# qazwsxal/diffusion-extensions

Measured on NVIDIA B200. Metric: igso3_score_evals_per_sec, higher is better.
Workload: dtype f32

## Files before the change

### diffusion_extensions_b200/csrc/so3d_kernels.cu

```cuda
#include <cuda_runtime.h>
#include <stdio.h>
#include <type_traits>
#include <stdlib.h>
#include <string.h>

#include "../../include/so3d.h"
#include "so3d_math.cuh"
#include "so3d_lanes.cuh"
#include "so3d_tma.cuh"
#include "so3d_cdf_smem.cuh"

using namespace so3d;

namespace {

constexpr int kTile = 256;

#ifndef SO3D_QS_OUTSTAGES
#define SO3D_QS_OUTSTAGES 1
#endif
#ifndef SO3D_QS_MINCTAS
#define SO3D_QS_MINCTAS 4
#endif
#ifndef SO3D_WROW_SHFL
// ... 1133 lines not shown
    float ga;
    aa_to_rmat_bwd(a3[0], angle[i], a9[0], &o3[0], &ga);
    g_angle[i] = ga;
  }
};
struct ExpVecBwdOp {
  SO3D_OP_ARRAYS(1, 1, 0, 1)
  SO3D_OP_NO_TAB
  __device__ void row(int64_t, const Mat3* a9, const Vec3* a3, Mat3*, Vec3* o3, const float*) const {
    o3[0] = exp_vec_bwd(a3[0], exp_vec(a3[0]), a9[0]);
  }
};
struct ScaleBwdOp {
  SO3D_OP_ARRAYS(2, 0, 1, 0)
  SO3D_OP_NO_TAB
  const float* s;
  int s_stride;
  float* g_s;
  __device__ void row(int64_t i, const Mat3* a9, const Vec3*, Mat3* o9, Vec3*, const float*) const {
    const float sc = s[i * s_stride];
    const Vec3 lv = log_vec(a9[0]);
    const Vec3 w{sc * lv.x, sc * lv.y, sc * lv.z};
    const Vec3 gw = exp_vec_bwd(w, exp_vec(w), a9[1]);
    if (g_s) g_s[i] = fmaf(lv.x, gw.x, fmaf(lv.y, gw.y, lv.z * gw.z));
    const Vec3 gl{0.5f * sc * gw.x, 0.5f * sc * gw.y, 0.5f * sc * gw.z};
    o9[0] = log_bwd(a9[0], hat(gl));
  }
};

#ifndef SO3D_LOGP_PREFETCH
#define SO3D_LOGP_PREFETCH 1
#endif
template <bool kOn>
struct LogpPre {};
template <>
struct LogpPre<true> {
  struct Pre1 {};
  struct Pre2 {
    float eps;
  };
};
template <int kMode>
struct LogpScoreOp : LogpPre<SO3D_LOGP_PREFETCH && (kMode == kClosed || kMode == kAuto)> {
  SO3D_OP_ARRAYS(1, 0, 0, 1)
  SO3D_OP_NO_TAB
  static constexpr int kMinCtas = (kMode == kClosed || kMode == kAuto) ? 5 : 1;
#ifndef SO3D_SERIES_WIDE_INDEX
#define SO3D_SERIES_WIDE_INDEX 0
#endif
  static constexpr bool kWideIndex = SO3D_SERIES_WIDE_INDEX && (kMode == kSeries || kMode == kSeriesAdaptive || kMode == kSeriesPure);
  const float* eps;
  int eps_stride;
  float* logp;
  float* dlogf;
  int L;
  __device__ void row(int64_t i, const Mat3* a9, const Vec3*, Mat3*, Vec3* o3, const float*) const { row_eps(i, eps[i * eps_stride], a9, o3); }
  __device__ void row_eps(int64_t i, float e, const Mat3* a9, Vec3* o3) const {
    const AxisAngleF a = axis_angle_fast(a9[0]);
    float lf, g;
    igso3_logf_g_t<kMode>(a.theta, e, L, &lf, &g);
    logp[i] = lf;
    if (dlogf) dlogf[i] = g;
    o3[0] = Vec3{g * a.axis.x, g * a.axis.y, g * a.axis.z};
  }
  template <class P1 = typename LogpPre<true>::Pre1>
  __device__ P1 prefetch1(int64_t) const { return P1{}; }
  template <class P1, class P2 = typename LogpPre<true>::Pre2>
  __device__ P2 prefetch2(int64_t i, const P1&) const { return P2{eps[i * eps_stride]}; }
  template <class P2>
  __device__ void row(int64_t i, const P2& p, const Mat3* a9, const Vec3*, Mat3*, Vec3* o3, const float*) const { row_eps(i, p.eps, a9, o3); }
};
#ifndef SO3D_LOGP2_MINCTAS
#define SO3D_LOGP2_MINCTAS 8
#endif
#ifndef SO3D_LOGP2_AUTO_VOTE
#define SO3D_LOGP2_AUTO_VOTE 1
#endif
#ifndef SO3D_LOGP2_OUTSTAGES
#define SO3D_LOGP2_OUTSTAGES 1
#endif
#ifndef SO3D_SERIES2_MINCTAS
#define SO3D_SERIES2_MINCTAS 4
#endif
template <int kMode>
struct LogpScore2Op : LogpScoreOp<kMode> {
  static constexpr bool kSeriesMode = kMode == kSeries || kMode == kSeriesAdaptive || kMode == kSeriesPure;
  using Pre1 = typename LogpPre<true>::Pre1;
  using Pre2 = typename LogpPre<true>::Pre2;
  static constexpr int kOutStages = SO3D_LOGP2_OUTSTAGES;
  static constexpr int kInStages = 1;
  static constexpr int kMinCtas = kSeriesMode ? SO3D_SERIES2_MINCTAS : SO3D_LOGP2_MINCTAS;
  int64_t n;
  __device__ void row2(int64_t i0, const Pre2 (&p)[2], const Mat3 (*a9)[2], const Vec3 (*)[2], Mat3 (*)[2], Vec3 (*o3)[2], const float*) const {
    const AxisAngleL<L2> a = axis_angle_fast_l(lanes_of(a9[0][0], a9[0][1]));
    float lf2[2], g2[2];
    if constexpr (kSeriesMode) {
      igso3_series_branch_l2<kMode>(a.theta, L2{p[0].eps, p[1].eps}, this->L, lf2, g2);
    } else if (kMode == kAuto && SO3D_LOGP2_AUTO_VOTE) {
      igso3_closed_f32(a.theta.x, p[0].eps, &lf2[0], &g2[0]);
      igso3_closed_f32(a.theta.y, p[1].eps, &lf2[1], &g2[1]);
      const bool s0 = !(p[0].eps <= kAutoSeriesEps), s1 = !(p[1].eps <= kAutoSeriesEps);
      if (__any_sync(__activemask(), s0 || s1)) {
        if (s0) igso3_series_branch<kAuto>(a.theta.x, p[0].eps, this->L, &lf2[0], &g2[0]);
        if (s1) igso3_series_branch<kAuto>(a.theta.y, p[1].eps, this->L, &lf2[1], &g2[1]);
      }
    } else {
      igso3_logf_g_t<kMode>(a.theta.x, p[0].eps, this->L, &lf2[0], &g2[0]);
      igso3_logf_g_t<kMode>(a.theta.y, p[1].eps, this->L, &lf2[1], &g2[1]);
    }
#pragma unroll
    for (int j = 0; j < 2; ++j) {
      const int64_t i = i0 + 32 * j;
      const float lf = lf2[j], g = g2[j];
      if (i < n) {
        this->logp[i] = lf;
        if (this->dlogf) this->dlogf[i] = g;
      }
      o3[0][j] = j ? Vec3{g * a.axis.x.y, g * a.axis.y.y, g * a.axis.z.y} : Vec3{g * a.axis.x.x, g * a.axis.y.x, g * a.axis.z.x};
    }
  }
};
struct LogpBwdOp {
  SO3D_OP_ARRAYS(1, 0, 1, 0)
  SO3D_OP_NO_TAB
  const float* dlogf;
  const float* gout;
  __device__ void row(int64_t i, const Mat3* a9, const Vec3*, Mat3* o9, Vec3*, const float*) const {
    const Mat3& r = a9[0];
    const float vx = r.m[7] - r.m[5], vy = r.m[2] - r.m[6], vz = r.m[3] - r.m[1];
    const float s = 0.5f * sqrtf(fmaf(vx, vx, fmaf(vy, vy, vz * vz)));
    const float c = 0.5f * (r.m[0] + r.m[4] + r.m[8] - 1.0f);
    const float gg = gout[i] * dlogf[i] / fmaf(s, s, c * c);
    const float ka = s > 0.f ? gg * c / (4.0f * s) : 0.f;
    const float kd = -0.5f * gg * s;
#pragma unroll
    for (int p = 0; p < 3; ++p)
#pragma unroll
      for (int q = 0; q < 3; ++q) o9[0].m[3 * p + q] = ka * (r.m[3 * p + q] - r.m[3 * q + p]) + (p == q ? kd : 0.f);
  }
};

__global__ void __launch_bounds__(256) density_kernel(const float* __restrict__ omega, const float* __restrict__ eps, int eps_stride,
                                                      float* __restrict__ f, int64_t n, int mode, int L) {
  for (int64_t i = (int64_t)blockIdx.x * blockDim.x + threadIdx.x; i < n; i += (int64_t)gridDim.x * blockDim.x) {
    float lf, g;
    igso3_logf_g(omega[i], eps[i * eps_stride], mode, L, &lf, &g);
    f[i] = expf(lf);
  }
}

template <int kMode>
__global__ void __launch_bounds__(256) series_warp_kernel(const float* __restrict__ R, const float* __restrict__ eps, int eps_stride,
                                                          float* __restrict__ logp, float* __restrict__ score3, float* __restrict__ dlogf,
                                                          int64_t n, int L) {
  const int lane = threadIdx.x & 31;
  const int64_t warps = ((int64_t)gridDim.x * blockDim.x) >> 5;
  for (int64_t row = ((int64_t)blockIdx.x * blockDim.x + threadIdx.x) >> 5; row < n; row += warps) {
    Mat3 m;
#pragma unroll
    for (int k = 0; k < 9; ++k) m.m[k] = __ldg(R + row * 9 + k);
    const AxisAngleF a = axis_angle_fast(m);
    const float e = __ldg(eps + row * eps_stride);
    float kap, kapp, cexp;
    igso3_series_lane_setup(a.theta, e, &kap, &kapp, &cexp);
    const int Lw = igso3_series_warp_terms(e, L);
    SeriesLaneState st = igso3_series_lane(kap, kapp, cexp, lane, igso3_series_lane_terms(Lw), Lw);
#pragma unroll
    for (int off = 16; off > 0; off >>= 1) {
      st.b += __shfl_xor_sync(0xffffffffu, st.b, off);
      st.d += __shfl_xor_sync(0xffffffffu, st.d, off);
      st.bp += __shfl_xor_sync(0xffffffffu, st.bp, off);
      st.dp += __shfl_xor_sync(0xffffffffu, st.dp, off);
    }
    if (lane == 0) {
      const float F = 2.0f * st.b - st.d, dF = 2.0f * st.bp - st.dp;
      float lf = logf(2.0f * F), g = dF / F;
      if ((kMode == kSeries || kMode == kSeriesAdaptive) && e <= kAutoSeriesEps && a.theta > kSeriesGuard * e) igso3_closed_f32(a.theta, e, &lf, &g);
      logp[row] = lf;
      if (dlogf) dlogf[row] = g;
      if (score3) {
// ... 1078 lines not shown
  op.in9[0] = R; op.q = q4;
  return launch_rowwise_pick(op, n, stream, "so3d_rmat_to_quat_f32");
}

}

template <bool TA, bool TB>
static int compose_dispatch(const float* A, int a_stride, const float* B, int b_stride, float* C, int64_t n, void* stream) {
  if (a_stride && b_stride) {
    ComposeOp<TA, TB> op;
    op.in9[0] = A; op.in9[1] = B; op.out9[0] = C;
    return launch_rowwise_pick(op, n, stream, "so3d_compose_f32");
  } else if (!a_stride && b_stride) {
    ComposeSharedOp<TA, TB, true> op;
    op.in9[0] = B; op.shared = A; op.out9[0] = C;
    return launch_rowwise_pick(op, n, stream, "so3d_compose_f32");
  } else if (a_stride && !b_stride) {
    ComposeSharedOp<TA, TB, false> op;
    op.in9[0] = A; op.shared = B; op.out9[0] = C;
    return launch_rowwise_pick(op, n, stream, "so3d_compose_f32");
  }
  return fail(SO3D_EINVAL, "so3d_compose_f32: at most one operand may be shared");
}

extern "C" {

int so3d_compose_f32(const float* A, int a_stride, int trans_a, const float* B, int b_stride, int trans_b, float* C,
                     int64_t n, void* stream) {
  SO3D_REQUIRE(n == 0 || (A && B && C), "so3d_compose_f32: null pointer");
  if (trans_a && trans_b) return compose_dispatch<true, true>(A, a_stride, B, b_stride, C, n, stream);
  if (trans_a) return compose_dispatch<true, false>(A, a_stride, B, b_stride, C, n, stream);
  if (trans_b) return compose_dispatch<false, true>(A, a_stride, B, b_stride, C, n, stream);
  return compose_dispatch<false, false>(A, a_stride, B, b_stride, C, n, stream);
}

int so3d_rmat_dist_f32(const float* A, const float* B, float* out, int64_t n, void* stream) {
  SO3D_REQUIRE(n == 0 || (A && B && out), "so3d_rmat_dist_f32: null pointer");
  RmatDistOp op;
  op.in9[0] = A; op.in9[1] = B; op.out = out;
  return launch_rowwise_pick(op, n, stream, "so3d_rmat_dist_f32", true);
}

int so3d_lerp_f32(const float* A, const float* B, const float* w, int w_stride, float* out, int64_t n, void* stream) {
  SO3D_REQUIRE(n == 0 || (A && B && w && out), "so3d_lerp_f32: null pointer");
  SO3D_REQUIRE(w_stride == 0 || w_stride == 1, "so3d_lerp_f32: w_stride must be 0 or 1");
  LerpOp op;
  op.in9[0] = A; op.in9[1] = B; op.w = w; op.w_stride = w_stride; op.out9[0] = out;
  return launch_rowwise_pick(op, n, stream, "so3d_lerp_f32");
}

int so3d_log_bwd_f32(const float* R, const float* G9, float* gR, int64_t n, void* stream) {
  SO3D_REQUIRE(n == 0 || (R && G9 && gR), "so3d_log_bwd_f32: null pointer");
  LogBwdOp op;
  op.in9[0] = R; op.in9[1] = G9; op.out9[0] = gR;
  return launch_rowwise_pick(op, n, stream, "so3d_log_bwd_f32");
}

int so3d_aa_to_rmat_bwd_f32(const float* axis3, const float* angle, const float* G9, float* g_axis3, float* g_angle,
                            int64_t n, void* stream) {
  SO3D_REQUIRE(n == 0 || (axis3 && angle && G9 && g_axis3 && g_angle), "so3d_aa_to_rmat_bwd_f32: null pointer");
  AaToRmatBwdOp op;
  op.in9[0] = G9; op.in3[0] = axis3; op.angle = angle; op.out3[0] = g_axis3; op.g_angle = g_angle;
  return launch_rowwise_pick(op, n, stream, "so3d_aa_to_rmat_bwd_f32");
}

int so3d_expvec_bwd_f32(const float* v3, const float* G9, float* g_v3, int64_t n, void* stream) {
  SO3D_REQUIRE(n == 0 || (v3 && G9 && g_v3), "so3d_expvec_bwd_f32: null pointer");
  ExpVecBwdOp op;
  op.in9[0] = G9; op.in3[0] = v3; op.out3[0] = g_v3;
  return launch_rowwise_pick(op, n, stream, "so3d_expvec_bwd_f32");
}

int so3d_scale_bwd_f32(const float* R, const float* s, int s_stride, const float* G9, float* gR, float* g_s, int64_t n,
                       void* stream) {
  SO3D_REQUIRE(n == 0 || (R && s && G9 && gR), "so3d_scale_bwd_f32: null pointer");
  SO3D_REQUIRE(s_stride == 0 || s_stride == 1, "so3d_scale_bwd_f32: s_stride must be 0 or 1");
  ScaleBwdOp op;
  op.in9[0] = R; op.in9[1] = G9; op.s = s; op.s_stride = s_stride; op.g_s = g_s; op.out9[0] = gR;
  return launch_rowwise_pick(op, n, stream, "so3d_scale_bwd_f32");
}

}

template <int kMode>
static int launch_logp_score(const float* R, const float* eps, int eps_stride, float* logp, float* score3, float* dlogf, int64_t n, int L,
                             void* stream) {
  constexpr bool kSeriesMode = LogpScore2Op<kMode>::kSeriesMode;
  if constexpr (kSeriesMode || SO3D_LOGP_PREFETCH) {
    const char* lanes_env = getenv("SO3D_LOGP_LANES");
    if (!(lanes_env && atoi(lanes_env) == 1)) {
      LogpScore2Op<kMode> op2;
      op2.in9[0] = R; op2.eps = eps; op2.eps_stride = eps_stride; op2.logp = logp; op2.dlogf = dlogf; op2.out3[0] = score3;
      op2.L = L; op2.n = n;
      return launch_rowwise_w2(op2, n, stream, "so3d_igso3_logp_score_f32", kMode == kSeriesAdaptive ? 3 : 0);
    }
  }
  LogpScoreOp<kMode> op;
  op.in9[0] = R; op.eps = eps; op.eps_stride = eps_stride; op.logp = logp; op.dlogf = dlogf; op.out3[0] = score3;
  op.L = L;
  const int ctas = (kMode == kSeries || kMode == kSeriesAdaptive || kMode == kSeriesPure) ? 3 : 0;
  return launch_rowwise(op, n, stream, "so3d_igso3_logp_score_f32", ctas);
}

extern "C" {

static int check_mode(int mode, int L) {
  if (mode < 0 || mode > 4) return fail(SO3D_EINVAL, "mode must be SO3D_MODE_{SERIES,CLOSED,AUTO,SERIES_ADAPTIVE,SERIES_PURE}");
  if (mode != SO3D_MODE_CLOSED && (L < 1 || L > 2896)) return fail(SO3D_EINVAL, "series truncation L must be in [1, 2896]");
  return 0;
}

int so3d_igso3_density_f32(const float* omega, const float* eps, int eps_stride, float* f, int64_t n, int mode, int L,
                           void* stream) {
  SO3D_REQUIRE(n >= 0, "negative n");
  if (n == 0) return 0;
  SO3D_REQUIRE(omega && eps && f, "so3d_igso3_density_f32: null pointer");
  SO3D_REQUIRE(eps_stride == 0 || eps_stride == 1, "eps_stride must be 0 or 1");
  if (int rc = check_mode(mode, L)) return rc;
  const int64_t blocks = (n + 255) / 256;
  const int64_t cap = (int64_t)sm_count() * 8;
  density_kernel<<<(int)(blocks < cap ? blocks : cap), 256, 0, (cudaStream_t)stream>>>(omega, eps, eps_stride, f, n, mode, L);
  return check_launch("so3d_igso3_density_f32");
}

int so3d_igso3_logp_score_f32(const float* R, const float* eps, int eps_stride, float* logp, float* score3, float* dlogf,
                              int64_t n, int mode, int L, void* stream) {
  SO3D_REQUIRE(n == 0 || (R && eps && logp), "so3d_igso3_logp_score_f32: null pointer");
  SO3D_REQUIRE(eps_stride == 0 || eps_stride == 1, "eps_stride must be 0 or 1");
  if (int rc = check_mode(mode, L)) return rc;
  if (n > 0 && (mode == SO3D_MODE_SERIES || mode == SO3D_MODE_SERIES_ADAPTIVE || mode == SO3D_MODE_SERIES_PURE)) {
    static const int64_t rows_per_sm = [] { const char* e = getenv("SO3D_SERIES_WARP_ROWS"); return e ? (int64_t)atoll(e) : (int64_t)64; }();
    if (n <= rows_per_sm * sm_count()) {
      const int64_t blocks = (n * 32 + 255) / 256;
      const int64_t cap = (int64_t)sm_count() * 8;
      const int grid = (int)(blocks < cap ? blocks : cap);
      if (mode == SO3D_MODE_SERIES_PURE)
        series_warp_kernel<kSeriesPure><<<grid, 256, 0, (cudaStream_t)stream>>>(R, eps, eps_stride, logp, score3, dlogf, n, L);
      else
        series_warp_kernel<kSeries><<<grid, 256, 0, (cudaStream_t)stream>>>(R, eps, eps_stride, logp, score3, dlogf, n, L);
      return check_launch("so3d_igso3_logp_score_f32");
    }
  }
  switch (mode) {
    case SO3D_MODE_SERIES: return launch_logp_score<kSeries>(R, eps, eps_stride, logp, score3, dlogf, n, L, stream);
    case SO3D_MODE_CLOSED: return launch_logp_score<kClosed>(R, eps, eps_stride, logp, score3, dlogf, n, L, stream);
    case SO3D_MODE_AUTO: return launch_logp_score<kAuto>(R, eps, eps_stride, logp, score3, dlogf, n, L, stream);
    case SO3D_MODE_SERIES_PURE: return launch_logp_score<kSeriesPure>(R, eps, eps_stride, logp, score3, dlogf, n, L, stream);
    default: return launch_logp_score<kSeriesAdaptive>(R, eps, eps_stride, logp, score3, dlogf, n, L, stream);
  }
}

int so3d_igso3_logp_bwd_f32(const float* R, const float* dlogf, const float* gout, float* gR, int64_t n, void* stream) {
  SO3D_REQUIRE(n == 0 || (R && dlogf && gout && gR), "so3d_igso3_logp_bwd_f32: null pointer");
  LogpBwdOp op;
  op.in9[0] = R; op.dlogf = dlogf; op.gout = gout; op.out9[0] = gR;
  return launch_rowwise_pick(op, n, stream, "so3d_igso3_logp_bwd_f32");
}

int so3d_igso3_cdf_table_f32(const float* eps, int64_t rows, const float* grid_loc, const float* haar_w, float* trap_out,
                             int quirks, void* stream) {
  SO3D_REQUIRE(rows >= 0, "negative rows");
  if (rows == 0) return 0;
  SO3D_REQUIRE(eps && grid_loc && haar_w && trap_out, "so3d_igso3_cdf_table_f32: null pointer");
  SO3D_REQUIRE(rows <= 0x7fffffff, "so3d_igso3_cdf_table_f32: too many rows");
  cdf_table_kernel<<<(int)rows, 256, 0, (cudaStream_t)stream>>>(eps, grid_loc, haar_w, trap_out, quirks);
  return check_launch("so3d_igso3_cdf_table_f32");
}

}

template <bool kShared>
static int launch_sample(const float* cdf, const uint32_t* guide, const float* loc, int64_t rows, const int64_t* row_idx, int64_t row,
                         const float* u, const float* axes3, uint64_t seed, uint64_t rng_offset, uint64_t row_offset, const float* mean,
                         int mean_stride, float* R, float* angle, float* axis3, int64_t n, void* stream) {
  SampleOp<kShared> op;
  op.out9[0] = R; op.out3[0] = axis3;
  op.cdf = cdf; op.guide = guide; op.loc = loc; op.row_idx = row_idx; op.shared_row = row; op.rows = rows; op.u_in = u; op.axes_in = axes3;
// ... 331 lines not shown
```

### diffusion_extensions_b200/csrc/so3d_lanes.cuh

```cuda
#pragma once

#include "so3d_math.cuh"

namespace so3d {

struct L1 {
  float x;
};
struct alignas(8) L2 {
  float x, y;
};
struct M1 {
  bool x;
};
struct M2 {
  bool x, y;
};
template <class L>
struct MaskOf;
template <>
struct MaskOf<L1> {
  using type = M1;
};
template <>
// ... 237 lines not shown
  const M pos = ge(n2, bc<L>(kFltMin));
  const L rs = sel(pos, vrsqrt(n2), zero);
  const L c = mulc(0.5f, add(add(add(r.m[0], r.m[4]), r.m[8]), bc<L>(-1.0f)));
  AxisAngleL<L> o;
  o.theta = atan2_pos_l(mul(mul(sel(tiny, bc<L>(0.5f * kTinyDown), bc<L>(0.5f)), n2), rs), c);
  const L d0 = sub(r.m[0], c), d1 = sub(r.m[4], c), d2 = sub(r.m[8], c);
  const L s01 = mulc(0.5f, add(r.m[1], r.m[3])), s02 = mulc(0.5f, add(r.m[2], r.m[6])), s12 = mulc(0.5f, add(r.m[5], r.m[7]));
  const M p0 = mand(ge(d0, d1), ge(d0, d2));
  const M p1 = ge(d1, d2);
  const L cx = sel(p0, d0, sel(p1, s01, s02));
  const L cy = sel(p0, s01, sel(p1, d1, s12));
  const L cz = sel(p0, s02, sel(p1, s12, d2));
  const L cn = vrsqrt(vmax(fma(cx, cx, fma(cy, cy, mul(cz, cz))), bc<L>(1e-30f)));
  const L sg = sel(lt(fma(cx, vx, fma(cy, vy, mul(cz, vz))), zero), neg(cn), cn);
  const M near_pi = lt(c, bc<L>(kNearPiCos));
  o.axis.x = sel(near_pi, mul(cx, sg), mul(vx, rs));
  o.axis.y = sel(near_pi, mul(cy, sg), mul(vy, rs));
  o.axis.z = sel(near_pi, mul(cz, sg), sel(mnot(pos), bc<L>(1.0f), mul(vz, rs)));
  return o;
}
template <class L>
SO3D_HD void quat_axis_halfangle_l(const QuatL<L>& q, Vec3L<L>* n, L* half) {
  using M = typename MaskOf<L>::type;
  const L zero = bc<L>(0.f);
  const M tiny = lt(fma(q.x, q.x, fma(q.y, q.y, mul(q.z, q.z))), bc<L>(kFltMin));
  const L sc = sel(tiny, bc<L>(kTinyUp), bc<L>(1.0f));
  const L x = mul(q.x, sc), y = mul(q.y, sc), z = mul(q.z, sc);
  const L v2 = fma(x, x, fma(y, y, mul(z, z)));
  const M pos = ge(v2, bc<L>(kFltMin));
  const L rs = sel(pos, vrsqrt(v2), zero);
  *half = atan2_pos_l(mul(mul(sel(tiny, bc<L>(kTinyDown), bc<L>(1.0f)), v2), rs), vabs(q.w));
  const L k = sel(lt(q.w, zero), neg(rs), rs);
  *n = Vec3L<L>{mul(x, k), mul(y, k), sel(pos, mul(z, k), bc<L>(1.0f))};
}

template <class L, bool kHasPred>
SO3D_HD QuatL<L> p_mean_quat_l(const Mat3L<L>& x_t, const Vec3L<L>& pred, float a, float b, float c1, float c2, QuatL<L>* x0h) {
  const AxisAngleL<L> ax = axis_angle_fast_l(x_t);
  QuatL<L> qh = quat_axis_angle_l(ax.axis, mulc(a, ax.theta));
  if (kHasPred) {
    const QuatL<L> q2 = quat_exp_vec_l(Vec3L<L>{mulc(-b, pred.x), mulc(-b, pred.y), mulc(-b, pred.z)});
    qh = qmul_l(qh, q2);
  }
  Vec3L<L> n0;
  L h0;
  quat_axis_halfangle_l(qh, &n0, &h0);
  const QuatL<L> q3 = quat_axis_angle_l(n0, mulc(2.0f * c1, h0));
  const QuatL<L> q4 = quat_axis_angle_l(ax.axis, mulc(c2, ax.theta));
  *x0h = qh;
  return qmul_l(q3, q4);
}

template <class L>
SO3D_HD QuatL<L> p_mean_quat_rows_l(const Mat3L<L>& x_t, const Vec3L<L>& pred, L a, L b, L c1, L c2, QuatL<L>* x0h) {
  const AxisAngleL<L> ax = axis_angle_fast_l(x_t);
  const L nb = neg(b);
  const QuatL<L> q1 = quat_axis_angle_l(ax.axis, mul(a, ax.theta));
  const QuatL<L> q2 = quat_exp_vec_l(Vec3L<L>{mul(nb, pred.x), mul(nb, pred.y), mul(nb, pred.z)});
  const QuatL<L> qh = qmul_l(q1, q2);
  Vec3L<L> n0;
  L h0;
  quat_axis_halfangle_l(qh, &n0, &h0);
  const QuatL<L> q3 = quat_axis_angle_l(n0, mul(mulc(2.0f, c1), h0));
  const QuatL<L> q4 = quat_axis_angle_l(ax.axis, mul(c2, ax.theta));
  *x0h = qh;
  return qmul_l(q3, q4);
}

SO3D_HD void sincos_draw_l(L1 x, L1* s, L1* c) { sincos_draw(x.x, &s->x, &c->x); }
SO3D_HD void sincos_draw_l(L2 x, L2* s, L2* c) {
  sincos_draw(x.x, &s->x, &c->x);
  sincos_draw(x.y, &s->y, &c->y);
}
template <class L>
SO3D_HD Vec3L<L> sphere_from_uniforms_l(L ua, L ub) {
  const L z = fma(bc<L>(-2.0f), ua, bc<L>(1.0f));
  const L t = mul(mulc(4.0f, ua), sub(bc<L>(1.0f), ua));
  const L r = mul(t, vrsqrt(vmax(t, bc<L>(1e-30f))));
  L sp, cp;
  sincos_draw_l(fma(bc<L>(kTwoPi), ub, bc<L>(-kPi)), &sp, &cp);
  return Vec3L<L>{mul(r, cp), mul(r, sp), z};
}

#ifndef SO3D_SERIES2_ORDER
#define SO3D_SERIES2_ORDER 0
#endif
#ifndef SO3D_SERIES2_BLOCK
#define SO3D_SERIES2_BLOCK 32
#endif
constexpr int kSeries2Block = SO3D_SERIES2_BLOCK;
struct SeriesStateL2 {
  L2 b, d, bp, dp, b2, bp2;
};
SO3D_HD L2 series_dsrc_l2(L2 kapp, L2 b, L2 dp) {
#if SO3D_SERIES_DERIV
  (void)kapp;
  return sub(dp, b);
#else
  return fnma(kapp, b, dp);
#endif
}
template <int kUnroll>
SO3D_HD void igso3_series_run_l2(SeriesStateL2& st, L2 kap, L2 kapp, L2 cexp, int hi, int count) {
#pragma unroll kUnroll
  for (int i = 0; i < count; ++i) {
    const int l = hi - i;
    const L2 e = vex2(mul(bc<L2>(series_mm(l)), cexp));
    const L2 mh = bc<L2>(series_mh(l));
    st.b2 = st.b;
    st.bp2 = st.bp;
#if SO3D_SERIES2_ORDER == 0
    const L2 dn = fnma(kap, st.b, fma(e, mh, st.d));
    const L2 dpn = fnma(kap, st.bp, series_dsrc_l2(kapp, st.b, st.dp));
    st.b = add(st.b, dn);
    st.bp = add(st.bp, dpn);
#elif SO3D_SERIES2_ORDER == 1
    const L2 t = fma(e, mh, st.d);
    const L2 u = series_dsrc_l2(kapp, st.b, st.dp);
    const L2 dn = fnma(kap, st.b, t);
    const L2 dpn = fnma(kap, st.bp, u);
    st.b = add(st.b, dn);
    st.bp = add(st.bp, dpn);
#elif SO3D_SERIES2_ORDER == 2
    const L2 dpn = fnma(kap, st.bp, series_dsrc_l2(kapp, st.b, st.dp));
    const L2 dn = fnma(kap, st.b, fma(e, mh, st.d));
    st.bp = add(st.bp, dpn);
    st.b = add(st.b, dn);
#else
    const L2 dn = fnma(kap, st.b, fma(e, mh, st.d));
    const L2 bn = add(st.b, dn);
    const L2 u = series_dsrc_l2(kapp, st.b, st.dp);
    const L2 dpn = fnma(kap, st.bp, u);
    st.b = bn;
    st.bp = add(st.bp, dpn);
#endif
    st.d = dn;
    st.dp = dpn;
  }
}

template <int kMode>
SO3D_HD void igso3_series_branch_l2(L2 w, L2 eps, int L, float* logf_out, float* g_out) {
  static_assert(kMode == kSeries || kMode == kSeriesAdaptive || kMode == kSeriesPure, "series modes only");
  int terms = L;
  if (kMode == kSeriesAdaptive) {
    const int t0 = igso3_series_live_terms(eps.x, L), t1 = igso3_series_live_terms(eps.y, L);
    terms = t0 > t1 ? t0 : t1;
#if defined(__CUDA_ARCH__)
    terms = __reduce_max_sync(__activemask(), terms);
#endif
#if SO3D_SERIES_ROUNDUP
    const int up = (terms + kSeries2Block - 1) / kSeries2Block * kSeries2Block;
    terms = up <= L ? up : L;
#endif
  }
  constexpr bool kGuarded = kMode != kSeriesPure;
  const bool guard0 = kGuarded && eps.x <= kAutoSeriesEps && w.x > kSeriesGuard * eps.x;
  const bool guard1 = kGuarded && eps.y <= kAutoSeriesEps && w.y > kSeriesGuard * eps.y;
  float lf_c[2] = {0.f, 0.f}, g_c[2] = {0.f, 0.f};
  if (guard0) igso3_closed_f32_outofline(w.x, eps.x, &lf_c[0], &g_c[0]);
  if (guard1) igso3_closed_f32_outofline(w.y, eps.y, &lf_c[1], &g_c[1]);
  L2 kap, kapp, cexp;
  igso3_series_lane_setup(w.x, eps.x, &kap.x, &kapp.x, &cexp.x);
  igso3_series_lane_setup(w.y, eps.y, &kap.y, &kapp.y, &cexp.y);
  const L2 zero = bc<L2>(0.f);
  SeriesStateL2 st{zero, zero, zero, zero, zero, zero};
  const int ragged = terms % kSeries2Block;
  if (ragged) igso3_series_run_l2<1>(st, kap, kapp, cexp, terms - 1, ragged);
  for (int blk = terms / kSeries2Block - 1; blk >= 0; --blk)
    igso3_series_run_l2<kSeries2Block>(st, kap, kapp, cexp, blk * kSeries2Block + (kSeries2Block - 1), kSeries2Block);
  const L2 F = add(st.b, st.b2);
#if SO3D_SERIES_DERIV
  const L2 dF = mul(kapp, add(st.bp, st.bp2));
#else
  const L2 dF = add(st.bp, st.bp2);
#endif
  logf_out[0] = guard0 ? lf_c[0] : logf(2.0f * F.x);
  g_out[0] = guard0 ? g_c[0] : dF.x / F.x;
  logf_out[1] = guard1 ? lf_c[1] : logf(2.0f * F.y);
  g_out[1] = guard1 ? g_c[1] : dF.y / F.y;
}

template <class L>
SO3D_HD QuatL<L> q_sample_quat_l(const Mat3L<L>& x0, L sc, const Vec3L<L>& axis, L ang, QuatL<L>* qn_out) {
  const QuatL<L> qn = quat_axis_angle_l(axis, ang);
  const AxisAngleL<L> ax = axis_angle_fast_l(x0);
  *qn_out = qn;
  return qmul_l(quat_axis_angle_l(ax.axis, mul(sc, ax.theta)), qn);
}

SO3D_HD Mat3L<L1> lanes_of(const Mat3& a) {
  Mat3L<L1> r;
  for (int k = 0; k < 9; ++k) r.m[k] = L1{a.m[k]};
  return r;
}
SO3D_HD Mat3L<L2> lanes_of(const Mat3& a, const Mat3& b) {
  Mat3L<L2> r;
  for (int k = 0; k < 9; ++k) r.m[k] = L2{a.m[k], b.m[k]};
  return r;
}

}
```

### profiles/sass_series_reads.py

```python
#!/usr/bin/env python
import argparse
import collections
import json
import os
import re
import subprocess
import sys

ROOT = os.path.dirname(os.path.dirname(os.path.abspath(__file__)))
sys.path.insert(0, ROOT)

WORDS_PER_CLK = 2.0
XU_CLK_PER_MUFU = 8.0
INS = re.compile(r"/\*([0-9a-f]{4,})\*/\s+(.*?)\s*;")
REG = re.compile(r"^-?\|?(R\d+)((?:\.\w+)*)\|?$")


def cuobjdump():
    from diffusion_extensions_b200 import build
    return os.path.join(os.path.dirname(build.find_nvcc()), "cuobjdump")


def functions(sass):
    out, cur = {}, None
    for line in sass.splitlines():
        if "Function :" in line:
            cur = out.setdefault(line.split("Function :")[1].strip(), [])
            continue
        m = INS.search(line)
        if cur is not None and m:
            cur.append((int(m.group(1), 16), m.group(2)))
    return out


def parse(text):
    t = re.sub(r"^@!?U?P\w+\s+", "", text)
    op, _, rest = t.partition(" ")
    ops = [o.strip() for o in rest.split(",")] if rest else []
    has_dst = not (op.startswith(("BRA", "EXIT", "RET", "BAR", "ST", "RED", "NOP", "WARPSYNC", "BSYNC", "CALL")))
    return op, ops[1:] if has_dst and ops else ops


def reads(src):
    r = []
    for slot, o in enumerate(src):
        m = REG.match(o)
        if not m:
            continue
        mods = m.group(2)
        r.append((slot, 2 if ".F32x2" in mods else 1, ".reuse" in mods))
    return r


def basic_blocks(ins):
    targets = {int(t, 16) for _, x in ins for t in re.findall(r"\bBRA(?:\.\w+)*\s+(?:!?U?P\w+,\s*)?(0x[0-9a-f]+)", x)}
    blocks, cur = [], []
    for addr, x in ins:
        if addr in targets and cur:
            blocks.append(cur)
            cur = []
        cur.append((addr, x))
        if re.search(r"\b(BRA|EXIT|RET|CALL)\b", x):
            blocks.append(cur)
            cur = []
    if cur:
        blocks.append(cur)
    return blocks


def count(block, rows):
    ops = collections.Counter()
    words = reused = mufu = 0
    for _, x in block:
        op, src = parse(x)
        ops[op] += 1
        if op.startswith("MUFU"):
            mufu += 1
        for _, w, ru in reads(src):
            words += w
            reused += w if ru else 0
    if not mufu:
        sys.exit("the block has no MUFU: not a series block")
    terms = mufu / rows
    per = lambda v: round(v / terms, 3)
    return {
        "terms_in_block": terms,
        "instructions_per_term": per(sum(ops.values())),
        "opcodes_per_term": {k: per(v) for k, v in sorted(ops.items(), key=lambda kv: -kv[1])},
        "mufu_per_term": per(mufu),
        "register_words_per_term": per(words),
        "reuse_words_per_term": per(reused),
        "read_floor_clk": per(words / WORDS_PER_CLK),
        "read_floor_clk_after_reuse": per((words - reused) / WORDS_PER_CLK),
        "xu_floor_clk": per(mufu * XU_CLK_PER_MUFU),
    }


def main():
    ap = argparse.ArgumentParser()
    ap.add_argument("lib", nargs="?", default=os.path.join(ROOT, "diffusion_extensions_b200", "libso3d.so"))
    ap.add_argument("--kernel", default=r"rowwise_kernel_w2INS_12LogpScore2OpILi0EEEE")
    ap.add_argument("--rows-per-thread", type=int, default=2)
    ap.add_argument("--json", action="store_true", help="one JSON line per kernel instead of the table")
    a = ap.parse_args()
    sass = subprocess.run([cuobjdump(), "-sass", a.lib], capture_output=True, text=True, check=True).stdout
    found = [(n, i) for n, i in functions(sass).items() if re.search(a.kernel, n)]
    if not found:
        sys.exit(f"no kernel matches {a.kernel!r} in {a.lib}")
    for name, ins in found:
        blk = max(basic_blocks(ins), key=lambda b: sum(1 for _, x in b if "MUFU.EX2" in x))
        r = {"lib": os.path.basename(a.lib), "kernel": name, "rows_per_term": a.rows_per_thread, **count(blk, a.rows_per_thread)}
        if a.json:
            print(json.dumps(r))
            continue
        print(f"{name}  ({r['lib']}, unrolled block of {r['terms_in_block']:g} terms of {a.rows_per_thread} rows)")
        print("  per term: " + ", ".join(f"{v:g} {k}" for k, v in r["opcodes_per_term"].items()))
        print(f"  register words {r['register_words_per_term']:g}, of which .reuse {r['reuse_words_per_term']:g};  "
              f"read floor {r['read_floor_clk']:g} clk ({r['read_floor_clk_after_reuse']:g} after reuse), XU floor {r['xu_floor_clk']:g} clk")


if __name__ == "__main__":
    main()
```

Before: 2.003 billion.

## Add warp-queue series kernel that compacts series rows and resolves closed-form rows inline

For large inputs in series mode, a new persistent kernel evaluates each row and writes it directly with the closed-form expression when eps is small and theta is above the guard. The remaining rows are compacted into a per-warp shared-memory queue, and the expensive series recurrence runs only on full 64-row batches, which removes divergence from mixed rows. It also selects a different statement order (order 3) for the series recurrence term, now chosen by template instead of a macro. The cost is extra shared-memory traffic, queue shuffling, and scattered output writes.

After: 2.458 billion (median of 6 runs). 22.7% higher.

```diff
diff --git a/diffusion_extensions_b200/csrc/so3d_kernels.cu b/diffusion_extensions_b200/csrc/so3d_kernels.cu
--- a/diffusion_extensions_b200/csrc/so3d_kernels.cu
+++ b/diffusion_extensions_b200/csrc/so3d_kernels.cu
@@ -1239,7 +1239,8 @@
 #ifndef SO3D_SERIES2_MINCTAS
 #define SO3D_SERIES2_MINCTAS 4
 #endif
-template <int kMode>
+constexpr int kSeriesWaveCtas = 6;
+template <int kMode, int kOrder = 0>
 struct LogpScore2Op : LogpScoreOp<kMode> {
   static constexpr bool kSeriesMode = kMode == kSeries || kMode == kSeriesAdaptive || kMode == kSeriesPure;
   using Pre1 = typename LogpPre<true>::Pre1;
@@ -1252,7 +1253,7 @@
     const AxisAngleL<L2> a = axis_angle_fast_l(lanes_of(a9[0][0], a9[0][1]));
     float lf2[2], g2[2];
     if constexpr (kSeriesMode) {
-      igso3_series_branch_l2<kMode>(a.theta, L2{p[0].eps, p[1].eps}, this->L, lf2, g2);
+      igso3_series_branch_l2<kMode, kOrder>(a.theta, L2{p[0].eps, p[1].eps}, this->L, lf2, g2);
     } else if (kMode == kAuto && SO3D_LOGP2_AUTO_VOTE) {
       igso3_closed_f32(a.theta.x, p[0].eps, &lf2[0], &g2[0]);
       igso3_closed_f32(a.theta.y, p[1].eps, &lf2[1], &g2[1]);
@@ -2497,6 +2498,126 @@
 
 }
 
+constexpr int kSeriesQThreads = 128;
+constexpr int kSeriesQCap = 128;
+constexpr int kSeriesQMinCtas = 7;
+template <int kOrder>
+__global__ void __launch_bounds__(kSeriesQThreads, kSeriesQMinCtas)
+    series_queue_kernel(const float* __restrict__ R, const float* __restrict__ eps, int eps_stride, float* __restrict__ logp,
+                        float* __restrict__ score3, float* __restrict__ dlogf, int64_t n, int L) {
+  constexpr int kWarps = kSeriesQThreads / 32;
+  __shared__ float q_w[kWarps][kSeriesQCap], q_e[kWarps][kSeriesQCap], q_x[kWarps][kSeriesQCap], q_y[kWarps][kSeriesQCap],
+      q_z[kWarps][kSeriesQCap];
+  __shared__ int64_t q_i[kWarps][kSeriesQCap];
+  const int lane = threadIdx.x & 31, wid = __shfl_sync(0xffffffffu, (int)threadIdx.x >> 5, 0);
+  float *qw = q_w[wid], *qe = q_e[wid], *qx = q_x[wid], *qy = q_y[wid], *qz = q_z[wid];
+  int64_t* qi = q_i[wid];
+  auto put = [&](int64_t i, float lf, float g, float ax, float ay, float az) {
+    logp[i] = lf;
+    if (dlogf) dlogf[i] = g;
+    if (score3) {
+      score3[i * 3] = g * ax;
+      score3[i * 3 + 1] = g * ay;
+      score3[i * 3 + 2] = g * az;
+    }
+  };
+  auto run_batch = [&](int count) {
+    const int k0 = lane, k1 = lane + 32;
+    const bool v0 = k0 < count, v1 = k1 < count;
+    const L2 w{v0 ? qw[k0] : 0.f, v1 ? qw[k1] : 0.f};
+    const L2 e{v0 ? qe[k0] : 1.f, v1 ? qe[k1] : 1.f};
+    float lf2[2], g2[2];
+    igso3_series_branch_l2<kSeriesPure, kOrder>(w, e, L, lf2, g2);
+    if (v0) put(qi[k0], lf2[0], g2[0], qx[k0], qy[k0], qz[k0]);
+    if (v1) put(qi[k1], lf2[1], g2[1], qx[k1], qy[k1], qz[k1]);
+  };
+  int count = 0;
+  const int64_t chunks = (n + 63) / 64;
+  const int64_t gw = (int64_t)blockIdx.x * kWarps + wid, nw = (int64_t)gridDim.x * kWarps;
+  for (int64_t c = gw; c < chunks; c += nw) {
+    const int64_t i0 = c * 64 + lane, i1 = i0 + 32;
+    const bool in0 = i0 < n, in1 = i1 < n;
+    Mat3 m0, m1;
+#pragma unroll
+    for (int t = 0; t < 9; ++t) {
+      m0.m[t] = in0 ? __ldg(R + i0 * 9 + t) : 1.f;
+      m1.m[t] = in1 ? __ldg(R + i1 * 9 + t) : 1.f;
+    }
+    const float e0 = in0 ? __ldg(eps + (eps_stride ? i0 : 0)) : 1.f, e1 = in1 ? __ldg(eps + (eps_stride ? i1 : 0)) : 1.f;
+    const AxisAngleL<L2> a = axis_angle_fast_l(lanes_of(m0, m1));
+    const bool g0 = e0 <= kAutoSeriesEps && a.theta.x > kSeriesGuard * e0;
+    const bool g1 = e1 <= kAutoSeriesEps && a.theta.y > kSeriesGuard * e1;
+    float lf, g;
+    if (in0 && g0) {
+      igso3_closed_f32_outofline(a.theta.x, e0, &lf, &g);
+      put(i0, lf, g, a.axis.x.x, a.axis.y.x, a.axis.z.x);
+    }
+    if (in1 && g1) {
+      igso3_closed_f32_outofline(a.theta.y, e1, &lf, &g);
+      put(i1, lf, g, a.axis.x.y, a.axis.y.y, a.axis.z.y);
+    }
+    const bool s0 = in0 && !g0, s1 = in1 && !g1;
+    const unsigned m0b = __ballot_sync(0xffffffffu, s0), m1b = __ballot_sync(0xffffffffu, s1);
+    const unsigned below = (1u << lane) - 1u;
+    if (s0) {
+      const int k = count + __popc(m0b & below);
+      qw[k] = a.theta.x, qe[k] = e0, qx[k] = a.axis.x.x, qy[k] = a.axis.y.x, qz[k] = a.axis.z.x, qi[k] = i0;
+    }
+    if (s1) {
+      const int k = count + __popc(m0b) + __popc(m1b & below);
+      qw[k] = a.theta.y, qe[k] = e1, qx[k] = a.axis.x.y, qy[k] = a.axis.y.y, qz[k] = a.axis.z.y, qi[k] = i1;
+    }
+    count = __shfl_sync(0xffffffffu, count + __popc(m0b) + __popc(m1b), 0);
+    __syncwarp();
+    if (count >= 64) {
+      run_batch(64);
+      __syncwarp();
+      count -= 64;
+      float t_w[2], t_e[2], t_x[2], t_y[2], t_z[2];
+      int64_t t_i[2];
+#pragma unroll
+      for (int h = 0; h < 2; ++h) {
+        const int k = 64 + lane + 32 * h;
+        if (lane + 32 * h < count) t_w[h] = qw[k], t_e[h] = qe[k], t_x[h] = qx[k], t_y[h] = qy[k], t_z[h] = qz[k], t_i[h] = qi[k];
+      }
+      __syncwarp();
+#pragma unroll
+      for (int h = 0; h < 2; ++h) {
+        const int k = lane + 32 * h;
+        if (k < count) qw[k] = t_w[h], qe[k] = t_e[h], qx[k] = t_x[h], qy[k] = t_y[h], qz[k] = t_z[h], qi[k] = t_i[h];
+      }
+      __syncwarp();
+    }
+  }
+  if (count > 0) run_batch(count);
+}
+
+template <int kOrder>
+static int launch_series_queue(const float* R, const float* eps, int eps_stride, float* logp, float* score3, float* dlogf, int64_t n,
+                               int L, void* stream) {
+  static int resident_dev[kMaxDevices] = {};
+  const int dev = current_device();
+  if (resident_dev[dev] == 0) {
+    int occ = 0;
+    if (cudaOccupancyMaxActiveBlocksPerMultiprocessor(&occ, series_queue_kernel<kOrder>, kSeriesQThreads, 0) != cudaSuccess || occ < 1) occ = 1;
+    resident_dev[dev] = occ;
+  }
+  const int64_t blocks = (n + 64 * (kSeriesQThreads / 32) - 1) / (64 * (kSeriesQThreads / 32));
+  const int64_t cap = (int64_t)sm_count() * resident_dev[dev];
+  series_queue_kernel<kOrder><<<(int)(blocks < cap ? blocks : cap), kSeriesQThreads, 0, (cudaStream_t)stream>>>(R, eps, eps_stride, logp, score3,
+                                                                                                              dlogf, n, L);
+  return check_launch("so3d_igso3_logp_score_f32");
+}
+
+template <int kMode, int kOrder>
+static int launch_logp_score_w2(const float* R, const float* eps, int eps_stride, float* logp, float* score3, float* dlogf, int64_t n,
+                                int L, void* stream) {
+  LogpScore2Op<kMode, kOrder> op2;
+  op2.in9[0] = R; op2.eps = eps; op2.eps_stride = eps_stride; op2.logp = logp; op2.dlogf = dlogf; op2.out3[0] = score3;
+  op2.L = L; op2.n = n;
+  return launch_rowwise_w2(op2, n, stream, "so3d_igso3_logp_score_f32", kMode == kSeriesAdaptive ? 3 : 0);
+}
+
 template <int kMode>
 static int launch_logp_score(const float* R, const float* eps, int eps_stride, float* logp, float* score3, float* dlogf, int64_t n, int L,
                              void* stream) {
@@ -2504,10 +2625,13 @@
   if constexpr (kSeriesMode || SO3D_LOGP_PREFETCH) {
     const char* lanes_env = getenv("SO3D_LOGP_LANES");
     if (!(lanes_env && atoi(lanes_env) == 1)) {
-      LogpScore2Op<kMode> op2;
-      op2.in9[0] = R; op2.eps = eps; op2.eps_stride = eps_stride; op2.logp = logp; op2.dlogf = dlogf; op2.out3[0] = score3;
-      op2.L = L; op2.n = n;
-      return launch_rowwise_w2(op2, n, stream, "so3d_igso3_logp_score_f32", kMode == kSeriesAdaptive ? 3 : 0);
+      if constexpr (kMode == kSeries || kMode == kSeriesPure) {
+        if (n >= (int64_t)sm_count() * kSeriesWaveCtas * kRows2) {
+          if (kMode == kSeries) return launch_series_queue<3>(R, eps, eps_stride, logp, score3, dlogf, n, L, stream);
+          return launch_logp_score_w2<kMode, 3>(R, eps, eps_stride, logp, score3, dlogf, n, L, stream);
+        }
+      }
+      return launch_logp_score_w2<kMode, 0>(R, eps, eps_stride, logp, score3, dlogf, n, L, stream);
     }
   }
   LogpScoreOp<kMode> op;
diff --git a/diffusion_extensions_b200/csrc/so3d_lanes.cuh b/diffusion_extensions_b200/csrc/so3d_lanes.cuh
--- a/diffusion_extensions_b200/csrc/so3d_lanes.cuh
+++ b/diffusion_extensions_b200/csrc/so3d_lanes.cuh
@@ -343,9 +343,6 @@
   return Vec3L<L>{mul(r, cp), mul(r, sp), z};
 }
 
-#ifndef SO3D_SERIES2_ORDER
-#define SO3D_SERIES2_ORDER 0
-#endif
 #ifndef SO3D_SERIES2_BLOCK
 #define SO3D_SERIES2_BLOCK 32
 #endif
@@ -361,46 +358,38 @@
   return fnma(kapp, b, dp);
 #endif
 }
-template <int kUnroll>
+template <int kOrder>
+SO3D_HD void igso3_series_term_l2(SeriesStateL2& st, L2 e, float mh, L2 kap, L2 kapp) {
+  static_assert(kOrder == 0 || kOrder == 3, "statement orders 0 and 3");
+  st.b2 = st.b;
+  st.bp2 = st.bp;
+  L2 dn, dpn;
+  if constexpr (kOrder == 0) {
+    dn = fnma(kap, st.b, fma(e, bc<L2>(mh), st.d));
+    dpn = fnma(kap, st.bp, series_dsrc_l2(kapp, st.b, st.dp));
+    st.b = add(st.b, dn);
+    st.bp = add(st.bp, dpn);
+  } else {
+    dn = fnma(kap, st.b, fma(e, bc<L2>(mh), st.d));
+    const L2 bn = add(st.b, dn);
+    const L2 u = series_dsrc_l2(kapp, st.b, st.dp);
+    dpn = fnma(kap, st.bp, u);
+    st.b = bn;
+    st.bp = add(st.bp, dpn);
+  }
+  st.d = dn;
+  st.dp = dpn;
+}
+template <int kUnroll, int kOrder>
 SO3D_HD void igso3_series_run_l2(SeriesStateL2& st, L2 kap, L2 kapp, L2 cexp, int hi, int count) {
 #pragma unroll kUnroll
   for (int i = 0; i < count; ++i) {
     const int l = hi - i;
-    const L2 e = vex2(mul(bc<L2>(series_mm(l)), cexp));
-    const L2 mh = bc<L2>(series_mh(l));
-    st.b2 = st.b;
-    st.bp2 = st.bp;
-#if SO3D_SERIES2_ORDER == 0
-    const L2 dn = fnma(kap, st.b, fma(e, mh, st.d));
-    const L2 dpn = fnma(kap, st.bp, series_dsrc_l2(kapp, st.b, st.dp));
-    st.b = add(st.b, dn);
-    st.bp = add(st.bp, dpn);
-#elif SO3D_SERIES2_ORDER == 1
-    const L2 t = fma(e, mh, st.d);
-    const L2 u = series_dsrc_l2(kapp, st.b, st.dp);
-    const L2 dn = fnma(kap, st.b, t);
-    const L2 dpn = fnma(kap, st.bp, u);
-    st.b = add(st.b, dn);
-    st.bp = add(st.bp, dpn);
-#elif SO3D_SERIES2_ORDER == 2
-    const L2 dpn = fnma(kap, st.bp, series_dsrc_l2(kapp, st.b, st.dp));
-    const L2 dn = fnma(kap, st.b, fma(e, mh, st.d));
-    st.bp = add(st.bp, dpn);
-    st.b = add(st.b, dn);
-#else
-    const L2 dn = fnma(kap, st.b, fma(e, mh, st.d));
-    const L2 bn = add(st.b, dn);
-    const L2 u = series_dsrc_l2(kapp, st.b, st.dp);
-    const L2 dpn = fnma(kap, st.bp, u);
-    st.b = bn;
-    st.bp = add(st.bp, dpn);
-#endif
-    st.d = dn;
-    st.dp = dpn;
+    igso3_series_term_l2<kOrder>(st, vex2(mul(bc<L2>(series_mm(l)), cexp)), series_mh(l), kap, kapp);
   }
 }
 
-template <int kMode>
+template <int kMode, int kOrder>
 SO3D_HD void igso3_series_branch_l2(L2 w, L2 eps, int L, float* logf_out, float* g_out) {
   static_assert(kMode == kSeries || kMode == kSeriesAdaptive || kMode == kSeriesPure, "series modes only");
   int terms = L;
@@ -427,9 +416,9 @@
   const L2 zero = bc<L2>(0.f);
   SeriesStateL2 st{zero, zero, zero, zero, zero, zero};
   const int ragged = terms % kSeries2Block;
-  if (ragged) igso3_series_run_l2<1>(st, kap, kapp, cexp, terms - 1, ragged);
+  if (ragged) igso3_series_run_l2<1, kOrder>(st, kap, kapp, cexp, terms - 1, ragged);
   for (int blk = terms / kSeries2Block - 1; blk >= 0; --blk)
-    igso3_series_run_l2<kSeries2Block>(st, kap, kapp, cexp, blk * kSeries2Block + (kSeries2Block - 1), kSeries2Block);
+    igso3_series_run_l2<kSeries2Block, kOrder>(st, kap, kapp, cexp, blk * kSeries2Block + (kSeries2Block - 1), kSeries2Block);
   const L2 F = add(st.b, st.b2);
 #if SO3D_SERIES_DERIV
   const L2 dF = mul(kapp, add(st.bp, st.bp2));
diff --git a/profiles/sass_series_reads.py b/profiles/sass_series_reads.py
--- a/profiles/sass_series_reads.py
+++ b/profiles/sass_series_reads.py
@@ -99,7 +99,7 @@
 def main():
     ap = argparse.ArgumentParser()
     ap.add_argument("lib", nargs="?", default=os.path.join(ROOT, "diffusion_extensions_b200", "libso3d.so"))
-    ap.add_argument("--kernel", default=r"rowwise_kernel_w2INS_12LogpScore2OpILi0EEEE")
+    ap.add_argument("--kernel", default=r"series_queue_kernelILi3EE")
     ap.add_argument("--rows-per-thread", type=int, default=2)
     ap.add_argument("--json", action="store_true", help="one JSON line per kernel instead of the table")
     a = ap.parse_args()
```
